# project-codeflare/instaslice

Measured on AMD Instinct MI355X. Metric: pods_scheduled_per_s, higher is better.
Workload: dtype fp32; 1 GPU; model=sleep-pod-partition-allocation, global_batch=698, parallelism=1-controller-shards+1-node-agents, partitioning=static-spx, backend=amdsmi, payload_kernel=False, full=False, cpu_affinity=120-127,248-255, payload_every=0, policy=packed-fit

## Files before the change

__graft_entry__.py:

```python

from __future__ import annotations


def build() -> None:
    import build_native

    build_native.build()

    import instaslice_amd
    import instaslice_amd.agent
    import instaslice_amd.controller
    from instaslice_amd.ops import _payload
    from instaslice_amd.smi import _partitiond

    print("build OK: instaslice_amd + _partitiond + _payload importable")


def smoke() -> None:
    from instaslice_amd.ops import _payload
    from instaslice_amd.runtime.cluster import Cluster
    from instaslice_amd.smi.native import NativeAmdSmi

    ndev = _payload.device_count()
    assert ndev > 0, "smoke() requires a GPU"

    smi = NativeAmdSmi()
    smi.init()
    gpus = smi.list_gpus()
    assert gpus, "no AMD GPUs enumerated via libamd_smi"
    g0 = gpus[0]
    print(
        f"gpu0: {g0.model} uuid={g0.uuid} mem={g0.memory_gb}GB "
        f"mode={g0.compute_mode}/{g0.memory_mode} partitions={len(g0.partitions)}"
    )

    cluster = Cluster(teardown_grace_s=0.0)
    cluster.add_node("smoke-node", smi)
    cluster.start()
    try:
        from instaslice_amd.partition.profiles import ProfileCatalog

        cr = cluster.store.get("Instaslice", "smoke-node", "instaslice-system")
        cat = ProfileCatalog.from_dict(cr["spec"]["placements"])
        profile = next(
            p for p in cat.profiles if p.compute.value == g0.compute_mode
        )
        cluster.submit_pod("smoke-pod", profile.name)
        cluster.wait_pod_scheduled("smoke-pod", timeout=30.0)
        env = cluster.pod_env("smoke-pod")
        device_index = int(env["HIP_VISIBLE_DEVICES"])
        print(f"pod scheduled; partition device_index={device_index} "
              f"uuid={env['ROCR_VISIBLE_DEVICES']}")

        err = _payload.run_vecadd(1 << 22, device=device_index)
        assert err == 0.0, f"vecadd max_err={err}"
        _payload.run_busy(20.0, device=device_index)
        info = _payload.device_info(device_index)
        print(f"payload OK on {info['gcn_arch']}: vecadd exact, "
              f"{info['cu_count']} CUs, {info['xcd_count_visible']} XCD(s) visible")

        cluster.delete_pod("smoke-pod")
        cluster.wait_pod_gone("smoke-pod", timeout=30.0)
        cluster.wait_allocations_empty("smoke-node", timeout=30.0)
    finally:
        cluster.stop()
    print("smoke OK: allocate -> run HIP payload in partition -> teardown")


if __name__ == "__main__":
    import sys

    if len(sys.argv) > 1 and sys.argv[1] == "smoke":
        smoke()
    else:
        build()
```

build_native.py:

```python
#!/usr/bin/env python3

from __future__ import annotations

import os
import subprocess
import sys
import sysconfig
from pathlib import Path

ROOT = Path(__file__).resolve().parent
ROCM = Path(os.environ.get("ROCM_PATH", "/opt/rocm"))
HIPCC = str(ROCM / "bin" / "hipcc")
CLANGXX = str(ROCM / "bin" / "amdclang++")
ARCH = os.environ.get("PYTORCH_ROCM_ARCH", "gfx950")
EXT = sysconfig.get_config_var("EXT_SUFFIX") or ".so"


def pybind_includes() -> list:
    import pybind11

    return [f"-I{pybind11.get_include()}", f"-I{sysconfig.get_paths()['include']}"]


def _srchash(sources: list, cmd_sig: str) -> str:
    import hashlib

    h = hashlib.sha256()
    h.update(cmd_sig.encode())
    for s in sources:
        h.update(Path(s).read_bytes())
    return h.hexdigest()


def newer(target: Path, sources: list, cmd_sig: str = "") -> bool:
    if not target.exists():
        return False
    sidecar = target.with_suffix(target.suffix + ".srchash")
    if not sidecar.exists():
        return False
    return sidecar.read_text().strip() == _srchash(sources, cmd_sig)


def record_hash(target: Path, sources: list, cmd_sig: str = "") -> None:
    sidecar = target.with_suffix(target.suffix + ".srchash")
    sidecar.write_text(_srchash(sources, cmd_sig) + "\n")


def run(cmd: list) -> None:
    print("+", " ".join(str(c) for c in cmd), flush=True)
    subprocess.run([str(c) for c in cmd], check=True, cwd=ROOT)


def build(force: bool = False) -> None:
    smi_dir = ROOT / "instaslice_amd" / "smi"
    ops_dir = ROOT / "instaslice_amd" / "ops"
    bin_dir = ROOT / "instaslice_amd" / "bin"
    bin_dir.mkdir(exist_ok=True)
    (bin_dir / "__init__.py").touch()

    common = ["-O2", "-std=c++17", "-fPIC", f"-I{ROCM}/include",
              f"-L{ROCM}/lib", f"-Wl,-rpath,{ROCM}/lib"]

    src = smi_dir / "csrc" / "partitiond_pybind.cpp"
    hdr = smi_dir / "csrc" / "partitiond_core.hpp"
    out = smi_dir / f"_partitiond{EXT}"
    if force or not newer(out, [src, hdr], "pybind"):
        run([CLANGXX, "-shared", *common, *pybind_includes(), src, "-lamd_smi", "-o", out])
        record_hash(out, [src, hdr], "pybind")

    src = smi_dir / "csrc" / "partitiond_main.cpp"
    out = bin_dir / "partitiond"
    if force or not newer(out, [src, hdr], "daemon"):
        run([CLANGXX, *common, src, "-lamd_smi", "-o", out])
        record_hash(out, [src, hdr], "daemon")

    src = ops_dir / "csrc" / "payload_pybind.hip"
    hdr = ops_dir / "csrc" / "payload_core.hpp"
    hdr_gemm = ops_dir / "csrc" / "payload_gemm.hpp"
    out = ops_dir / f"_payload{EXT}"
    if force or not newer(out, [src, hdr, hdr_gemm], ARCH):
        run([HIPCC, f"--offload-arch={ARCH}", "-shared", *common,
             *pybind_includes(), src, "-o", out])
        record_hash(out, [src, hdr, hdr_gemm], ARCH)

    src = ops_dir / "csrc" / "payload_main.hip"
    out = bin_dir / "instaslice-payload"
    if force or not newer(out, [src, hdr, hdr_gemm], ARCH):
        run([HIPCC, f"--offload-arch={ARCH}", *common, src, "-o", out])
        record_hash(out, [src, hdr, hdr_gemm], ARCH)

    store_dir = ROOT / "instaslice_amd" / "store"
    src = store_dir / "csrc" / "stored_main.cpp"
    hdr2 = store_dir / "csrc" / "msgpack_value.hpp"
    out = bin_dir / "instaslice-stored"
    if force or not newer(out, [src, hdr2], "stored"):
        run(["g++", "-O2", "-std=c++17", "-pthread", src, "-o", out])
        record_hash(out, [src, hdr2], "stored")

    print("native build complete")


if __name__ == "__main__":
    build(force="--force" in sys.argv)
```

instaslice_amd/store/netstore.py:

```python

from __future__ import annotations

import queue
import socket
import socketserver
import struct
import threading
from typing import Callable, List, Optional, Tuple

import msgpack

from instaslice_amd.store.memstore import (
    AlreadyExists,
    Conflict,
    MemStore,
    NotFound,
)
from instaslice_amd.utils import get_logger

_EXC_BY_NAME = {
    "Conflict": Conflict,
    "NotFound": NotFound,
    "AlreadyExists": AlreadyExists,
}

_LEN = struct.Struct(">I")


def _pack(obj: dict) -> bytes:
    payload = msgpack.packb(obj, use_bin_type=True)
    return _LEN.pack(len(payload)) + payload


def _read_msg(rfile) -> Optional[dict]:
    hdr = rfile.read(4)
    if len(hdr) < 4:
        return None
    (n,) = _LEN.unpack(hdr)
    payload = rfile.read(n)
    if len(payload) < n:
        return None
    return msgpack.unpackb(payload, raw=False)


def _execute(store: MemStore, req: dict):
    verb = req.get("verb")
    if verb == "create":
        return store.create(req["obj"])
    if verb == "get":
        return store.get(req["kind"], req["name"], req.get("namespace", ""))
    if verb == "list":
        return store.list(req["kind"], req.get("namespace"))
    if verb == "update":
        return store.update(req["obj"])
    if verb == "delete":
        store.delete(req["kind"], req["name"], req.get("namespace", ""))
        return None
    if verb == "patch":
        return store.patch(req["kind"], req["name"], req.get("namespace", ""),
                           req.get("ops"))
    if verb == "ping":
        return "pong"
    raise ValueError(f"unknown verb {verb!r}")


class _Handler(socketserver.StreamRequestHandler):
    disable_nagle_algorithm = True

    def handle(self) -> None:
        store: MemStore = self.server.store
        log = self.server.log
        wlock = threading.Lock()
        watches = []

        def send(obj: dict) -> None:
            data = _pack(obj)
            with wlock:
                self.wfile.write(data)
                self.wfile.flush()

        def pump_watch(watch_id: int, w) -> None:
            while True:
                ev = w.next(timeout=0.5)
                if ev is None:
                    if w._stopped or self.server.stopping:
                        return
                    continue
                try:
                    send({"watch_id": watch_id, "event": list(ev)})
                except (BrokenPipeError, OSError, ValueError):
                    w.stop()
                    return

        next_watch_id = 0
        try:
            while True:
                req = _read_msg(self.rfile)
                if req is None:
                    break
                rid = req.get("id")
                verb = req.get("verb")
                quiet = req.get("quiet", False)
                try:
                    if verb == "batch":
                        res = store.batch(req["requests"], quiet=quiet)
                    elif verb == "watch":
                        w = store.watch(req.get("kind"), replay=req.get("replay", True),
                                        filters=req.get("filters"),
                                        since=req.get("since"))
                        watches.append(w)
                        next_watch_id += 1
                        wid = next_watch_id
                        send({"id": rid, "ok": True, "result": {
                            "watch_id": wid,
                            "rev": getattr(w, "rev", None),
                            "resumed": getattr(w, "resumed", False)}})
                        threading.Thread(
                            target=pump_watch, args=(wid, w), daemon=True
                        ).start()
                        continue
                    else:
                        res = _execute(store, req)
                        if quiet:
                            res = None
                    send({"id": rid, "ok": True, "result": res})
                except (Conflict, NotFound, AlreadyExists) as e:
                    send({"id": rid, "ok": False,
                          "error": {"type": type(e).__name__, "msg": str(e)}})
                except Exception as e:
                    log.warning("request error: %s", e)
                    send({"id": rid, "ok": False,
                          "error": {"type": "Error", "msg": str(e)}})
        except (ConnectionResetError, BrokenPipeError, OSError):
            pass
        finally:
            for w in watches:
                w.stop()


class StoreServer:

    def __init__(self, store: Optional[MemStore] = None,
                 host: str = "127.0.0.1", port: int = 0) -> None:
        self.store = store or MemStore()
        self.log = get_logger("netstore.server")
        self._srv = socketserver.ThreadingTCPServer((host, port), _Handler,
                                                    bind_and_activate=True)
        self._srv.daemon_threads = True
        self._srv.allow_reuse_address = True
        self._srv.store = self.store
        self._srv.log = self.log
        self._srv.stopping = False
        self.host, self.port = self._srv.server_address
        self._thread = threading.Thread(target=self._srv.serve_forever,
                                        name="netstore-server", daemon=True)

    def start(self) -> "StoreServer":
        self._thread.start()
        return self

    def stop(self) -> None:
        self._srv.stopping = True
        self._srv.shutdown()
        self._srv.server_close()


class _ClientWatch:

    def __init__(self) -> None:
        self._q: "queue.Queue[Optional[Tuple[str, dict]]]" = queue.Queue()
        self._stopped = False
        self.kind: Optional[str] = None
        self._cb = None
        self._cb_lock = threading.Lock()
        self.last_rev: Optional[int] = None

    def set_callback(self, fn) -> None:
        with self._cb_lock:
            while True:
                try:
                    ev = self._q.get_nowait()
                except queue.Empty:
                    break
                if ev is not None:
                    fn(*ev)
            self._cb = fn

    def _deliver(self, event) -> None:
        if self._stopped:
            return
        try:
            rv = int(event[1]["metadata"]["resourceVersion"])
            if self.last_rev is None or rv > self.last_rev:
                self.last_rev = rv
        except (KeyError, TypeError, ValueError, IndexError):
            pass
        with self._cb_lock:
            if self._cb is not None:
                try:
                    self._cb(*event)
                except Exception:
                    import traceback

                    traceback.print_exc()
                return
        self._q.put(event)

    def next(self, timeout: Optional[float] = None) -> Optional[Tuple[str, dict]]:
        try:
            return self._q.get(timeout=timeout)
        except queue.Empty:
            return None

    def stop(self) -> None:
        self._stopped = True
        self._q.put(None)


class NetStoreClient:

    def __init__(self, host: str, port: int, timeout: float = 30.0,
                 reconnect: bool = False,
                 reconnect_backoff_s: float = 0.2) -> None:
        self.host, self.port = host, port
        self._reconnect = reconnect
        self._reconnect_backoff_s = reconnect_backoff_s
        self._sock = socket.create_connection((host, port), timeout=timeout)
        self._sock.settimeout(None)
        self._sock.setsockopt(socket.IPPROTO_TCP, socket.TCP_NODELAY, 1)
        self._rfile = self._sock.makefile("rb")
        self._wlock = threading.Lock()
        self._pending: dict = {}
        self._watches: dict = {}
        self._watch_specs: dict = {}
        self._orphan_events: dict = {}
        self._watch_reg_lock = threading.Lock()
        self._next_id = 0
        self._idlock = threading.Lock()
        self._closed = False
        self.log = get_logger("netstore.client")
        self._reader = threading.Thread(target=self._read_loop,
                                        name="netstore-reader", daemon=True)
        self._reader.start()

    def _dispatch(self, msg: dict) -> None:
        if "watch_id" in msg and "event" in msg:
            wid = msg["watch_id"]
            et, obj = msg["event"]
            with self._watch_reg_lock:
                w = self._watches.get(wid)
                if w is None:
                    self._orphan_events.setdefault(wid, []).append((et, obj))
            if w is not None:
                w._deliver((et, obj))
            return
        ev = self._pending.pop(msg.get("id"), None)
        if ev is not None:
            ev[1] = msg
            ev[0].set()

    def _fail_pending(self, why: str) -> None:
        for rid in list(self._pending):
            ev = self._pending.pop(rid, None)
            if ev is not None:
                ev[1] = {"ok": False, "error": {"type": "Error", "msg": why}}
                ev[0].set()

    def _read_loop(self) -> None:
        while True:
            try:
                while True:
                    msg = _read_msg(self._rfile)
                    if msg is None:
                        break
                    self._dispatch(msg)
            except (OSError, ValueError):
                pass
            self._fail_pending("connection lost")
            if self._closed or not self._reconnect:
                break
            if not self._reconnect_once():
                break
        self._closed = True
        self._fail_pending("connection closed")
        for w in self._watches.values():
            w.stop()

    def _reconnect_once(self) -> bool:
        try:
            self._sock.close()
        except OSError:
            pass
        delay = self._reconnect_backoff_s
        while not self._closed:
            try:
                sock = socket.create_connection((self.host, self.port),
                                                timeout=5.0)
            except OSError:
                import time as _time

                _time.sleep(delay)
                delay = min(delay * 2, 5.0)
                continue
            sock.settimeout(None)
            sock.setsockopt(socket.IPPROTO_TCP, socket.TCP_NODELAY, 1)
            with self._wlock:
                self._sock = sock
                self._rfile = sock.makefile("rb")
            self._fail_pending("connection lost")
            with self._watch_reg_lock:
                live = [(w, spec) for (w, spec) in self._watch_specs.values()
                        if not w._stopped]
                self._watches = {}
            new_specs = {}
            ok = True
            for w, spec in live:
                with self._idlock:
                    self._next_id += 1
                    rid = self._next_id
                resync = dict(spec, replay=True)
                if w.last_rev is not None:
                    resync["since"] = w.last_rev
                try:
                    with self._wlock:
                        self._sock.sendall(_pack({"id": rid, "verb": "watch",
                                                  **resync}))
                    while True:
                        msg = _read_msg(self._rfile)
                        if msg is None:
                            ok = False
                            break
                        if msg.get("id") == rid:
                            new_wid = msg["result"]["watch_id"]
                            with self._watch_reg_lock:
                                self._watches[new_wid] = w
                            new_specs[new_wid] = (w, spec)
                            break
                        self._dispatch(msg)
                except (OSError, ValueError, KeyError):
                    ok = False
                if not ok:
                    break
            if ok:
                with self._watch_reg_lock:
                    self._watch_specs = new_specs
                self.log.warning(
                    "reconnected to store %s:%d (%d watches resynced)",
                    self.host, self.port, len(live))
                return True
            with self._watch_reg_lock:
                self._watches = {}
        return False

    def _call(self, verb: str, **kw):
        if self._closed:
            raise ConnectionError("netstore client closed")
        with self._idlock:
            self._next_id += 1
            rid = self._next_id
        ev = [threading.Event(), None]
        self._pending[rid] = ev
        req = _pack({"id": rid, "verb": verb, **kw})
        try:
            with self._wlock:
                self._sock.sendall(req)
        except OSError as e:
            self._pending.pop(rid, None)
            raise ConnectionError(f"netstore send failed: {e}") from e
        if not ev[0].wait(timeout=60.0):
            self._pending.pop(rid, None)
            raise TimeoutError(f"netstore call {verb} timed out")
        msg = ev[1]
        if msg["ok"]:
            return msg.get("result")
        err = msg["error"]
        if err["type"] == "Error" and "connection" in err["msg"]:
            raise ConnectionError(err["msg"])
        raise _EXC_BY_NAME.get(err["type"], RuntimeError)(err["msg"])


    def create(self, obj: dict) -> dict:
        return self._call("create", obj=obj)

    def get(self, kind: str, name: str, namespace: str = "") -> dict:
        return self._call("get", kind=kind, name=name, namespace=namespace)

    def list(self, kind: str, namespace: Optional[str] = None) -> List[dict]:
        return self._call("list", kind=kind, namespace=namespace)

    def update(self, obj: dict) -> dict:
        return self._call("update", obj=obj)

    def delete(self, kind: str, name: str, namespace: str = "", *, now: float = 0.0) -> None:
        self._call("delete", kind=kind, name=name, namespace=namespace)

    def patch(self, kind: str, name: str, namespace: str = "",
              ops: Optional[List[dict]] = None, *, quiet: bool = False):
        return self._call("patch", kind=kind, name=name, namespace=namespace,
                          ops=ops, quiet=quiet)

    def batch(self, requests: List[dict], *, quiet: bool = False) -> List[dict]:
        return self._call("batch", requests=requests, quiet=quiet)

    def watch(self, kind: Optional[str] = None, *, replay: bool = True,
              filters: Optional[List[dict]] = None):
        w = _ClientWatch()
        w.kind = kind
        spec = {"kind": kind, "replay": replay, "filters": filters}
        res = self._call("watch", kind=kind, replay=replay, filters=filters)
        wid = res["watch_id"]
        if isinstance(res, dict) and res.get("rev") is not None:
            w.last_rev = int(res["rev"])
        with self._watch_reg_lock:
            self._watches[wid] = w
            self._watch_specs[wid] = (w, spec)
            orphans = self._orphan_events.pop(wid, [])
        for ev in orphans:
            w._deliver(ev)
        return w

    def update_with_retry(
        self, kind: str, name: str, namespace: str,
        mutate: Callable[[dict], Optional[dict]], attempts: int = 25,
    ) -> Optional[dict]:
        for attempt in range(attempts):
            try:
                obj = self.get(kind, name, namespace)
            except NotFound:
                return None
            new = mutate(obj)
            if new is None:
                return None
            try:
                return self.update(new)
            except Conflict:
                if attempt >= 2:
                    import random
                    import time as _time

                    _time.sleep(random.random() * 0.002 * attempt)
                continue
        raise Conflict(f"update_with_retry: {attempts} attempts exhausted for {kind}/{name}")

    def close(self) -> None:
        self._closed = True
        try:
            self._sock.close()
        except OSError:
            pass
```

Measured before the change: 1000 pods/s.

## Add native C++ wire client for netstore RPC and event dispatch

Moves the netstore client's socket framing, msgpack encoding, response matching and reader thread into a pybind11 C++ extension. Request/response waits then happen in C++ condition variables instead of Python Events, and events are batched to Python callbacks. It is enabled by default when the extension builds. The aim is to cut Python GIL and per-message overhead on controller/agent store calls. In exchange it adds a new reconnect path and extra concurrency complexity.

New measurement: 1055 pods/s, median of 6. 1.06x the previous value.

```diff
diff --git a/__graft_entry__.py b/__graft_entry__.py
--- a/__graft_entry__.py
+++ b/__graft_entry__.py
@@ -12,8 +12,9 @@
     import instaslice_amd.controller
     from instaslice_amd.ops import _payload
     from instaslice_amd.smi import _partitiond
+    from instaslice_amd.store import _netclient
 
-    print("build OK: instaslice_amd + _partitiond + _payload importable")
+    print("build OK: instaslice_amd + _partitiond + _payload + _netclient importable")
 
 
 def smoke() -> None:
diff --git a/build_native.py b/build_native.py
--- a/build_native.py
+++ b/build_native.py
@@ -97,6 +97,14 @@
         run(["g++", "-O2", "-std=c++17", "-pthread", src, "-o", out])
         record_hash(out, [src, hdr2], "stored")
 
+    src = store_dir / "csrc" / "netclient_pybind.cpp"
+    hdr3 = store_dir / "csrc" / "netclient_core.hpp"
+    out = store_dir / f"_netclient{EXT}"
+    if force or not newer(out, [src, hdr3], "netclient"):
+        run(["g++", "-O2", "-std=c++17", "-fPIC", "-shared", "-pthread",
+             "-fvisibility=hidden", *pybind_includes(), src, "-o", out])
+        record_hash(out, [src, hdr3], "netclient")
+
     print("native build complete")
 
 
diff --git a/instaslice_amd/store/csrc/netclient_core.hpp b/instaslice_amd/store/csrc/netclient_core.hpp
--- /dev/null
+++ b/instaslice_amd/store/csrc/netclient_core.hpp
@@ -0,0 +1,489 @@
+
+#pragma once
+
+#include <sys/socket.h>
+#include <sys/types.h>
+
+#include <atomic>
+#include <cerrno>
+#include <chrono>
+#include <condition_variable>
+#include <cstdint>
+#include <cstring>
+#include <memory>
+#include <mutex>
+#include <string>
+#include <thread>
+#include <unordered_map>
+#include <utility>
+#include <vector>
+
+namespace netclient {
+
+constexpr uint32_t kMaxFrame = 64u << 20;
+
+
+struct Peek {
+  enum Kind { Response, Event, Other, Bad };
+  Kind kind = Bad;
+  uint64_t id = 0;
+};
+
+class Scanner {
+ public:
+  Scanner(const uint8_t* p, size_t n) : p_(p), end_(p + n) {}
+
+  bool at_end() const { return p_ == end_; }
+
+  bool skip() {
+    uint64_t todo = 1;
+    while (todo > 0) {
+      --todo;
+      if (p_ >= end_) return false;
+      uint8_t c = *p_++;
+      uint64_t n = 0;
+      if (c < 0x80 || c >= 0xe0) continue;
+      if ((c & 0xf0) == 0x80) { n = 2ull * (c & 0x0f); goto container; }
+      if ((c & 0xf0) == 0x90) { n = c & 0x0f; goto container; }
+      if ((c & 0xe0) == 0xa0) { if (!advance(c & 0x1f)) return false; continue; }
+      switch (c) {
+        case 0xc0: case 0xc2: case 0xc3: continue;
+        case 0xc4: case 0xd9: if (!take_be(1, n) || !advance(n)) return false; continue;
+        case 0xc5: case 0xda: if (!take_be(2, n) || !advance(n)) return false; continue;
+        case 0xc6: case 0xdb: if (!take_be(4, n) || !advance(n)) return false; continue;
+        case 0xca: case 0xce: case 0xd2: if (!advance(4)) return false; continue;
+        case 0xcb: case 0xcf: case 0xd3: if (!advance(8)) return false; continue;
+        case 0xcc: case 0xd0: if (!advance(1)) return false; continue;
+        case 0xcd: case 0xd1: if (!advance(2)) return false; continue;
+        case 0xdc: if (!take_be(2, n)) return false; goto container;
+        case 0xdd: if (!take_be(4, n)) return false; goto container;
+        case 0xde: if (!take_be(2, n)) return false; n *= 2; goto container;
+        case 0xdf: if (!take_be(4, n)) return false; n *= 2; goto container;
+        default: return false;
+      }
+    container:
+      todo += n;
+      if (todo > static_cast<uint64_t>(end_ - p_)) return false;
+    }
+    return true;
+  }
+
+  bool take_map(uint64_t& n) {
+    if (p_ >= end_) return false;
+    uint8_t c = *p_;
+    if ((c & 0xf0) == 0x80) { ++p_; n = c & 0x0f; return true; }
+    if (c == 0xde) { ++p_; return take_be(2, n); }
+    if (c == 0xdf) { ++p_; return take_be(4, n); }
+    return false;
+  }
+
+  bool take_str(const uint8_t*& s, size_t& len) {
+    if (p_ >= end_) return false;
+    uint8_t c = *p_;
+    uint64_t n = 0;
+    const uint8_t* save = p_;
+    if ((c & 0xe0) == 0xa0) { ++p_; n = c & 0x1f; }
+    else if (c == 0xd9) { ++p_; if (!take_be(1, n)) { p_ = save; return false; } }
+    else if (c == 0xda) { ++p_; if (!take_be(2, n)) { p_ = save; return false; } }
+    else if (c == 0xdb) { ++p_; if (!take_be(4, n)) { p_ = save; return false; } }
+    else return false;
+    if (static_cast<uint64_t>(end_ - p_) < n) { p_ = save; return false; }
+    s = p_;
+    len = static_cast<size_t>(n);
+    p_ += n;
+    return true;
+  }
+
+  bool take_uint(uint64_t& v) {
+    if (p_ >= end_) return false;
+    uint8_t c = *p_;
+    const uint8_t* save = p_;
+    if (c < 0x80) { ++p_; v = c; return true; }
+    int w = c == 0xcc ? 1 : c == 0xcd ? 2 : c == 0xce ? 4 : c == 0xcf ? 8 : 0;
+    int sw = c == 0xd0 ? 1 : c == 0xd1 ? 2 : c == 0xd2 ? 4 : c == 0xd3 ? 8 : 0;
+    if (w) {
+      ++p_;
+      if (!take_be(w, v)) { p_ = save; return false; }
+      return true;
+    }
+    if (sw) {
+      ++p_;
+      uint64_t raw;
+      if (!take_be(sw, raw)) { p_ = save; return false; }
+      if ((raw >> (8 * sw - 1)) & 1) { p_ = save; return false; }
+      v = raw;
+      return true;
+    }
+    return false;
+  }
+
+ private:
+  bool advance(uint64_t n) {
+    if (static_cast<uint64_t>(end_ - p_) < n) return false;
+    p_ += n;
+    return true;
+  }
+  bool take_be(int n, uint64_t& v) {
+    if (end_ - p_ < n) return false;
+    v = 0;
+    for (int k = 0; k < n; ++k) v = (v << 8) | *p_++;
+    return true;
+  }
+
+  const uint8_t* p_;
+  const uint8_t* end_;
+};
+
+inline Peek peek_frame(const uint8_t* p, size_t n) {
+  Peek out;
+  Scanner sc(p, n);
+  uint64_t pairs = 0;
+  if (!sc.take_map(pairs)) {
+    out.kind = (sc.skip() && sc.at_end()) ? Peek::Other : Peek::Bad;
+    return out;
+  }
+  bool has_id = false, has_wid = false, has_event = false;
+  uint64_t id = 0, wid = 0;
+  for (uint64_t k = 0; k < pairs; ++k) {
+    const uint8_t* s = nullptr;
+    size_t len = 0;
+    if (sc.take_str(s, len)) {
+      if (len == 2 && std::memcmp(s, "id", 2) == 0) {
+        uint64_t v;
+        if (sc.take_uint(v)) { has_id = true; id = v; continue; }
+        has_id = false;
+      } else if (len == 8 && std::memcmp(s, "watch_id", 8) == 0) {
+        uint64_t v;
+        if (sc.take_uint(v)) { has_wid = true; wid = v; continue; }
+        has_wid = false;
+      } else if (len == 5 && std::memcmp(s, "event", 5) == 0) {
+        has_event = true;
+      }
+    } else if (!sc.skip()) {
+      return out;
+    }
+    if (!sc.skip()) return out;
+  }
+  if (!sc.at_end()) return out;
+  if (has_wid && has_event) { out.kind = Peek::Event; out.id = wid; }
+  else if (has_id) { out.kind = Peek::Response; out.id = id; }
+  else out.kind = Peek::Other;
+  return out;
+}
+
+
+struct EventSink {
+  virtual ~EventSink() = default;
+  virtual bool on_events(std::vector<std::string>& frames) = 0;
+  virtual void on_lost(const char* why) = 0;
+};
+
+enum class Status { Ok, Pending, Timeout, Lost, Closed, SendFailed };
+
+inline const char* status_message(Status s) {
+  switch (s) {
+    case Status::Lost: return "connection lost";
+    case Status::Closed: return "connection closed";
+    case Status::Timeout: return "timed out";
+    case Status::SendFailed: return "send failed";
+    default: return "";
+  }
+}
+
+class Wire : public std::enable_shared_from_this<Wire> {
+  struct Waiter {
+    std::condition_variable cv;
+    bool done = false;
+    Status st = Status::Pending;
+    std::string frame;
+  };
+
+ public:
+  struct Stats {
+    uint64_t responses = 0;
+    uint64_t events = 0;
+    uint64_t dropped = 0;
+    uint64_t batches = 0;
+  };
+
+  static std::shared_ptr<Wire> create(int fd, std::shared_ptr<EventSink> sink) {
+    return std::shared_ptr<Wire>(new Wire(fd, std::move(sink)));
+  }
+
+  Wire(const Wire&) = delete;
+  Wire& operator=(const Wire&) = delete;
+
+  ~Wire() {
+    if (reader_.joinable()) {
+      if (reader_.get_id() == std::this_thread::get_id()) reader_.detach();
+      else reader_.join();
+    }
+  }
+
+  void start() {
+    std::lock_guard<std::mutex> g(join_mu_);
+    if (started_) return;
+    started_ = true;
+    auto self = shared_from_this();
+    reader_ = std::thread([self] { self->run(); });
+  }
+
+  class Call {
+   public:
+    Call(Wire& w, uint64_t id) : w_(w), id_(id) {
+      std::lock_guard<std::mutex> g(w_.mu_);
+      if (w_.lost_) {
+        wt_.done = true;
+        wt_.st = w_.lost_status_;
+      } else {
+        registered_ = w_.pending_.emplace(id_, &wt_).second;
+        if (!registered_) {
+          wt_.done = true;
+          wt_.st = Status::SendFailed;
+          err_ = EINVAL;
+        }
+      }
+    }
+    ~Call() {
+      if (!registered_) return;
+      std::lock_guard<std::mutex> g(w_.mu_);
+      auto it = w_.pending_.find(id_);
+      if (it != w_.pending_.end() && it->second == &wt_) w_.pending_.erase(it);
+    }
+    Call(const Call&) = delete;
+    Call& operator=(const Call&) = delete;
+
+    Status send(const char* data, size_t n) {
+      {
+        std::lock_guard<std::mutex> g(w_.mu_);
+        if (wt_.done) return wt_.st;
+      }
+      int e = w_.send_all(data, n);
+      if (e == 0) return Status::Ok;
+      std::lock_guard<std::mutex> g(w_.mu_);
+      if (wt_.done && wt_.st != Status::Ok) return wt_.st;
+      if (e < 0) return w_.stopping_.load() ? Status::Closed : Status::Lost;
+      err_ = e;
+      return Status::SendFailed;
+    }
+
+    Status wait_for(std::chrono::nanoseconds slice) {
+      std::unique_lock<std::mutex> g(w_.mu_);
+      if (!wt_.done) {
+#if defined(__SANITIZE_THREAD__)
+        wt_.cv.wait_until(g, std::chrono::system_clock::now() + slice,
+                          [&] { return wt_.done; });
+#else
+        wt_.cv.wait_for(g, slice, [&] { return wt_.done; });
+#endif
+      }
+      return wt_.done ? wt_.st : Status::Pending;
+    }
+
+    std::string& frame() { return wt_.frame; }
+    int send_errno() const { return err_; }
+
+   private:
+    Wire& w_;
+    uint64_t id_;
+    Waiter wt_;
+    bool registered_ = false;
+    int err_ = 0;
+  };
+
+  Status call(const std::string& framed_request, uint64_t id, double timeout_s,
+              std::string* response) {
+    Call c(*this, id);
+    Status st = c.send(framed_request.data(), framed_request.size());
+    if (st != Status::Ok) return st;
+    auto deadline = std::chrono::steady_clock::now() +
+                    std::chrono::duration_cast<std::chrono::nanoseconds>(
+                        std::chrono::duration<double>(timeout_s));
+    for (;;) {
+      auto now = std::chrono::steady_clock::now();
+      if (now >= deadline) return Status::Timeout;
+      st = c.wait_for(deadline - now);
+      if (st == Status::Pending) continue;
+      if (st == Status::Ok && response) *response = std::move(c.frame());
+      return st;
+    }
+  }
+
+  void stop() {
+    if (!stopping_.exchange(true))
+      ::shutdown(fd_, SHUT_RDWR);
+    {
+      std::lock_guard<std::mutex> g(write_mu_);
+      fd_dead_ = true;
+    }
+    bool joined = false;
+    {
+      std::lock_guard<std::mutex> g(join_mu_);
+      if (!started_) {
+        started_ = true;
+        joined = true;
+      } else if (reader_.joinable() &&
+                 reader_.get_id() != std::this_thread::get_id()) {
+        reader_.join();
+        joined = true;
+      }
+    }
+    if (joined) fail_all(Status::Closed);
+  }
+
+  void abort_connection() {
+    std::lock_guard<std::mutex> g(write_mu_);
+    if (!fd_dead_) ::shutdown(fd_, SHUT_RDWR);
+  }
+
+  bool alive() const {
+    std::lock_guard<std::mutex> g(mu_);
+    return !lost_;
+  }
+
+  Stats stats() const {
+    Stats s;
+    s.responses = responses_.load(std::memory_order_relaxed);
+    s.events = events_.load(std::memory_order_relaxed);
+    s.dropped = dropped_.load(std::memory_order_relaxed);
+    s.batches = batches_.load(std::memory_order_relaxed);
+    return s;
+  }
+
+  size_t pending() const {
+    std::lock_guard<std::mutex> g(mu_);
+    return pending_.size();
+  }
+
+ private:
+  Wire(int fd, std::shared_ptr<EventSink> sink) : fd_(fd), sink_(std::move(sink)) {}
+
+  int send_all(const char* p, size_t left) {
+    std::lock_guard<std::mutex> g(write_mu_);
+    if (fd_dead_) return -1;
+    while (left > 0) {
+      ssize_t n = ::send(fd_, p, left, MSG_NOSIGNAL);
+      if (n < 0) {
+        if (errno == EINTR) continue;
+        return errno ? errno : EIO;
+      }
+      p += n;
+      left -= static_cast<size_t>(n);
+    }
+    return 0;
+  }
+
+  void complete(uint64_t id, const uint8_t* p, size_t n) {
+    std::lock_guard<std::mutex> g(mu_);
+    auto it = pending_.find(id);
+    if (it == pending_.end()) {
+      dropped_.fetch_add(1, std::memory_order_relaxed);
+      return;
+    }
+    Waiter* w = it->second;
+    pending_.erase(it);
+    w->frame.assign(reinterpret_cast<const char*>(p), n);
+    w->st = Status::Ok;
+    w->done = true;
+    w->cv.notify_one();
+    responses_.fetch_add(1, std::memory_order_relaxed);
+  }
+
+  void fail_all(Status st) {
+    std::lock_guard<std::mutex> g(mu_);
+    if (!lost_) {
+      lost_ = true;
+      lost_status_ = st;
+    }
+    for (auto& kv : pending_) {
+      kv.second->st = st;
+      kv.second->done = true;
+      kv.second->cv.notify_one();
+    }
+    pending_.clear();
+  }
+
+  void run() {
+    std::vector<char> buf(64 * 1024);
+    size_t rd = 0, wr = 0;
+    std::vector<std::string> events;
+    while (!stopping_.load()) {
+      if (wr == buf.size()) {
+        if (rd > 0) {
+          std::memmove(buf.data(), buf.data() + rd, wr - rd);
+          wr -= rd;
+          rd = 0;
+        } else {
+          buf.resize(buf.size() * 2);
+        }
+      }
+      ssize_t n = ::recv(fd_, buf.data() + wr, buf.size() - wr, 0);
+      if (n < 0 && errno == EINTR) continue;
+      if (n <= 0) break;
+      wr += static_cast<size_t>(n);
+
+      bool bad = false;
+      while (wr - rd >= 4) {
+        const uint8_t* h = reinterpret_cast<const uint8_t*>(buf.data() + rd);
+        uint32_t len = (static_cast<uint32_t>(h[0]) << 24) | (static_cast<uint32_t>(h[1]) << 16) |
+                       (static_cast<uint32_t>(h[2]) << 8) | static_cast<uint32_t>(h[3]);
+        if (len > kMaxFrame) { bad = true; break; }
+        size_t need = 4 + static_cast<size_t>(len);
+        if (wr - rd < need) {
+          if (buf.size() - rd < need) {
+            std::memmove(buf.data(), buf.data() + rd, wr - rd);
+            wr -= rd;
+            rd = 0;
+            if (buf.size() < need) buf.resize(need);
+          }
+          break;
+        }
+        const uint8_t* f = h + 4;
+        Peek pk = peek_frame(f, len);
+        if (pk.kind == Peek::Response) complete(pk.id, f, len);
+        else if (pk.kind == Peek::Event) events.emplace_back(reinterpret_cast<const char*>(f), len);
+        else if (pk.kind == Peek::Other) dropped_.fetch_add(1, std::memory_order_relaxed);
+        else { bad = true; break; }
+        rd += need;
+      }
+      if (!events.empty()) {
+        events_.fetch_add(events.size(), std::memory_order_relaxed);
+        batches_.fetch_add(1, std::memory_order_relaxed);
+        bool ok = sink_ ? sink_->on_events(events) : true;
+        events.clear();
+        if (!ok) bad = true;
+      }
+      if (bad) break;
+      if (rd == wr) {
+        rd = wr = 0;
+        if (buf.size() > (1u << 20)) {
+          buf.resize(64 * 1024);
+          buf.shrink_to_fit();
+        }
+      }
+    }
+    bool closed = stopping_.load();
+    fail_all(closed ? Status::Closed : Status::Lost);
+    if (sink_) sink_->on_lost(status_message(closed ? Status::Closed : Status::Lost));
+  }
+
+  const int fd_;
+  std::shared_ptr<EventSink> sink_;
+
+  mutable std::mutex mu_;
+  std::unordered_map<uint64_t, Waiter*> pending_;
+  bool lost_ = false;
+  Status lost_status_ = Status::Lost;
+
+  std::mutex write_mu_;
+  bool fd_dead_ = false;
+
+  std::mutex join_mu_;
+  bool started_ = false;
+  std::thread reader_;
+  std::atomic<bool> stopping_{false};
+
+  std::atomic<uint64_t> responses_{0}, events_{0}, dropped_{0}, batches_{0};
+};
+
+}
diff --git a/instaslice_amd/store/csrc/netclient_pybind.cpp b/instaslice_amd/store/csrc/netclient_pybind.cpp
--- /dev/null
+++ b/instaslice_amd/store/csrc/netclient_pybind.cpp
@@ -0,0 +1,475 @@
+
+#include <pybind11/pybind11.h>
+
+#include <string>
+#include <vector>
+
+#include "netclient_core.hpp"
+
+namespace py = pybind11;
+using netclient::Status;
+using netclient::Wire;
+
+namespace {
+
+
+constexpr int kMaxDepth = 511;
+
+inline void put_be(std::string& out, uint64_t v, int n) {
+  for (int s = 8 * (n - 1); s >= 0; s -= 8) out.push_back(static_cast<char>(v >> s));
+}
+
+inline void put_uint(std::string& out, uint64_t n) {
+  if (n < 0x80) out.push_back(static_cast<char>(n));
+  else if (n <= 0xff) { out.push_back(static_cast<char>(0xcc)); put_be(out, n, 1); }
+  else if (n <= 0xffff) { out.push_back(static_cast<char>(0xcd)); put_be(out, n, 2); }
+  else if (n <= 0xffffffffULL) { out.push_back(static_cast<char>(0xce)); put_be(out, n, 4); }
+  else { out.push_back(static_cast<char>(0xcf)); put_be(out, n, 8); }
+}
+
+inline void put_int(std::string& out, int64_t v) {
+  if (v >= 0) { put_uint(out, static_cast<uint64_t>(v)); return; }
+  uint64_t u = static_cast<uint64_t>(v);
+  if (v >= -32) out.push_back(static_cast<char>(v));
+  else if (v >= INT8_MIN) { out.push_back(static_cast<char>(0xd0)); put_be(out, u, 1); }
+  else if (v >= INT16_MIN) { out.push_back(static_cast<char>(0xd1)); put_be(out, u, 2); }
+  else if (v >= INT32_MIN) { out.push_back(static_cast<char>(0xd2)); put_be(out, u, 4); }
+  else { out.push_back(static_cast<char>(0xd3)); put_be(out, u, 8); }
+}
+
+bool encode_obj(PyObject* o, std::string& out, int depth) {
+  if (o == Py_None) { out.push_back(static_cast<char>(0xc0)); return true; }
+  if (o == Py_True) { out.push_back(static_cast<char>(0xc3)); return true; }
+  if (o == Py_False) { out.push_back(static_cast<char>(0xc2)); return true; }
+  if (PyUnicode_CheckExact(o)) {
+    Py_ssize_t n = 0;
+    const char* s = PyUnicode_AsUTF8AndSize(o, &n);
+    if (!s) { PyErr_Clear(); return false; }
+    if (n < 32) out.push_back(static_cast<char>(0xa0 | n));
+    else if (n <= 0xff) { out.push_back(static_cast<char>(0xd9)); put_be(out, n, 1); }
+    else if (n <= 0xffff) { out.push_back(static_cast<char>(0xda)); put_be(out, n, 2); }
+    else if (static_cast<uint64_t>(n) <= 0xffffffffULL) { out.push_back(static_cast<char>(0xdb)); put_be(out, n, 4); }
+    else return false;
+    out.append(s, static_cast<size_t>(n));
+    return true;
+  }
+  if (PyLong_CheckExact(o)) {
+    int overflow = 0;
+    long long v = PyLong_AsLongLongAndOverflow(o, &overflow);
+    if (overflow == 0) {
+      if (v == -1 && PyErr_Occurred()) { PyErr_Clear(); return false; }
+      put_int(out, v);
+      return true;
+    }
+    if (overflow < 0) return false;
+    unsigned long long u = PyLong_AsUnsignedLongLong(o);
+    if (u == static_cast<unsigned long long>(-1) && PyErr_Occurred()) { PyErr_Clear(); return false; }
+    put_uint(out, u);
+    return true;
+  }
+  if (PyDict_CheckExact(o)) {
+    if (depth >= kMaxDepth) return false;
+    Py_ssize_t n = PyDict_Size(o);
+    if (n < 16) out.push_back(static_cast<char>(0x80 | n));
+    else if (n <= 0xffff) { out.push_back(static_cast<char>(0xde)); put_be(out, n, 2); }
+    else if (static_cast<uint64_t>(n) <= 0xffffffffULL) { out.push_back(static_cast<char>(0xdf)); put_be(out, n, 4); }
+    else return false;
+    Py_ssize_t pos = 0;
+    PyObject *k, *v;
+    while (PyDict_Next(o, &pos, &k, &v)) {
+      if (!encode_obj(k, out, depth + 1)) return false;
+      if (!encode_obj(v, out, depth + 1)) return false;
+    }
+    return true;
+  }
+  if (PyList_CheckExact(o) || PyTuple_CheckExact(o)) {
+    if (depth >= kMaxDepth) return false;
+    bool is_list = PyList_CheckExact(o);
+    Py_ssize_t n = is_list ? PyList_GET_SIZE(o) : PyTuple_GET_SIZE(o);
+    if (n < 16) out.push_back(static_cast<char>(0x90 | n));
+    else if (n <= 0xffff) { out.push_back(static_cast<char>(0xdc)); put_be(out, n, 2); }
+    else if (static_cast<uint64_t>(n) <= 0xffffffffULL) { out.push_back(static_cast<char>(0xdd)); put_be(out, n, 4); }
+    else return false;
+    for (Py_ssize_t i = 0; i < n; ++i) {
+      PyObject* e = is_list ? PyList_GET_ITEM(o, i) : PyTuple_GET_ITEM(o, i);
+      if (!encode_obj(e, out, depth + 1)) return false;
+    }
+    return true;
+  }
+  if (PyFloat_CheckExact(o)) {
+    double d = PyFloat_AS_DOUBLE(o);
+    uint64_t bits;
+    static_assert(sizeof(bits) == sizeof(d), "double size");
+    std::memcpy(&bits, &d, sizeof(bits));
+    out.push_back(static_cast<char>(0xcb));
+    put_be(out, bits, 8);
+    return true;
+  }
+  if (PyBytes_CheckExact(o)) {
+    Py_ssize_t n = PyBytes_GET_SIZE(o);
+    if (n <= 0xff) { out.push_back(static_cast<char>(0xc4)); put_be(out, n, 1); }
+    else if (n <= 0xffff) { out.push_back(static_cast<char>(0xc5)); put_be(out, n, 2); }
+    else if (static_cast<uint64_t>(n) <= 0xffffffffULL) { out.push_back(static_cast<char>(0xc6)); put_be(out, n, 4); }
+    else return false;
+    out.append(PyBytes_AS_STRING(o), static_cast<size_t>(n));
+    return true;
+  }
+  return false;
+}
+
+void encode_into(py::handle o, std::string& out) {
+  size_t mark = out.size();
+  if (encode_obj(o.ptr(), out, 0)) return;
+  out.resize(mark);
+  static py::object* packb = nullptr;
+  if (!packb) packb = new py::object(py::module_::import("msgpack").attr("packb"));
+  py::object b = (*packb)(o, py::arg("use_bin_type") = true);
+  char* p = nullptr;
+  Py_ssize_t n = 0;
+  if (PyBytes_AsStringAndSize(b.ptr(), &p, &n) != 0) throw py::error_already_set();
+  out.append(p, static_cast<size_t>(n));
+}
+
+
+struct Decoder {
+  const uint8_t* p;
+  const uint8_t* end;
+
+  PyObject* fail(const char* what) {
+    PyErr_SetString(PyExc_ValueError, what);
+    return nullptr;
+  }
+
+  bool take_be(int n, uint64_t& v) {
+    if (end - p < n) { fail("msgpack: incomplete input"); return false; }
+    v = 0;
+    for (int k = 0; k < n; ++k) v = (v << 8) | *p++;
+    return true;
+  }
+
+  PyObject* take_str(uint64_t n) {
+    if (static_cast<uint64_t>(end - p) < n) return fail("msgpack: incomplete input");
+    PyObject* s = PyUnicode_DecodeUTF8(reinterpret_cast<const char*>(p),
+                                       static_cast<Py_ssize_t>(n), nullptr);
+    p += n;
+    return s;
+  }
+
+  PyObject* take_bin(uint64_t n) {
+    if (static_cast<uint64_t>(end - p) < n) return fail("msgpack: incomplete input");
+    PyObject* b = PyBytes_FromStringAndSize(reinterpret_cast<const char*>(p),
+                                            static_cast<Py_ssize_t>(n));
+    p += n;
+    return b;
+  }
+
+  PyObject* take_arr(uint64_t n, int depth) {
+    if (static_cast<uint64_t>(end - p) < n) return fail("msgpack: incomplete input");
+    PyObject* l = PyList_New(static_cast<Py_ssize_t>(n));
+    if (!l) return nullptr;
+    for (uint64_t k = 0; k < n; ++k) {
+      PyObject* e = next(depth + 1);
+      if (!e) { Py_DECREF(l); return nullptr; }
+      PyList_SET_ITEM(l, static_cast<Py_ssize_t>(k), e);
+    }
+    return l;
+  }
+
+  PyObject* take_map(uint64_t n, int depth) {
+    if (static_cast<uint64_t>(end - p) / 2 < n) return fail("msgpack: incomplete input");
+    PyObject* d = PyDict_New();
+    if (!d) return nullptr;
+    for (uint64_t k = 0; k < n; ++k) {
+      PyObject* key = next(depth + 1);
+      if (!key) { Py_DECREF(d); return nullptr; }
+      if (!PyUnicode_CheckExact(key) && !PyBytes_CheckExact(key)) {
+        PyErr_Format(PyExc_ValueError, "%.100s is not allowed for map key",
+                     Py_TYPE(key)->tp_name);
+        Py_DECREF(key);
+        Py_DECREF(d);
+        return nullptr;
+      }
+      PyObject* val = next(depth + 1);
+      if (!val) { Py_DECREF(key); Py_DECREF(d); return nullptr; }
+      int rc = PyDict_SetItem(d, key, val);
+      Py_DECREF(key);
+      Py_DECREF(val);
+      if (rc != 0) { Py_DECREF(d); return nullptr; }
+    }
+    return d;
+  }
+
+  PyObject* next(int depth) {
+    if (depth > kMaxDepth) return fail("msgpack: nesting too deep");
+    if (p >= end) return fail("msgpack: incomplete input");
+    uint8_t c = *p++;
+    uint64_t n = 0;
+    if (c < 0x80) return PyLong_FromLong(c);
+    if (c >= 0xe0) return PyLong_FromLong(static_cast<int8_t>(c));
+    if ((c & 0xf0) == 0x80) return take_map(c & 0x0f, depth);
+    if ((c & 0xf0) == 0x90) return take_arr(c & 0x0f, depth);
+    if ((c & 0xe0) == 0xa0) return take_str(c & 0x1f);
+    switch (c) {
+      case 0xc0: Py_RETURN_NONE;
+      case 0xc2: Py_RETURN_FALSE;
+      case 0xc3: Py_RETURN_TRUE;
+      case 0xc4: return take_be(1, n) ? take_bin(n) : nullptr;
+      case 0xc5: return take_be(2, n) ? take_bin(n) : nullptr;
+      case 0xc6: return take_be(4, n) ? take_bin(n) : nullptr;
+      case 0xca: {
+        if (!take_be(4, n)) return nullptr;
+        uint32_t bits = static_cast<uint32_t>(n);
+        float f;
+        std::memcpy(&f, &bits, sizeof(f));
+        return PyFloat_FromDouble(f);
+      }
+      case 0xcb: {
+        if (!take_be(8, n)) return nullptr;
+        double d;
+        std::memcpy(&d, &n, sizeof(d));
+        return PyFloat_FromDouble(d);
+      }
+      case 0xcc: return take_be(1, n) ? PyLong_FromUnsignedLongLong(n) : nullptr;
+      case 0xcd: return take_be(2, n) ? PyLong_FromUnsignedLongLong(n) : nullptr;
+      case 0xce: return take_be(4, n) ? PyLong_FromUnsignedLongLong(n) : nullptr;
+      case 0xcf: return take_be(8, n) ? PyLong_FromUnsignedLongLong(n) : nullptr;
+      case 0xd0: return take_be(1, n) ? PyLong_FromLong(static_cast<int8_t>(n)) : nullptr;
+      case 0xd1: return take_be(2, n) ? PyLong_FromLong(static_cast<int16_t>(n)) : nullptr;
+      case 0xd2: return take_be(4, n) ? PyLong_FromLong(static_cast<int32_t>(n)) : nullptr;
+      case 0xd3: return take_be(8, n) ? PyLong_FromLongLong(static_cast<int64_t>(n)) : nullptr;
+      case 0xd9: return take_be(1, n) ? take_str(n) : nullptr;
+      case 0xda: return take_be(2, n) ? take_str(n) : nullptr;
+      case 0xdb: return take_be(4, n) ? take_str(n) : nullptr;
+      case 0xdc: return take_be(2, n) ? take_arr(n, depth) : nullptr;
+      case 0xdd: return take_be(4, n) ? take_arr(n, depth) : nullptr;
+      case 0xde: return take_be(2, n) ? take_map(n, depth) : nullptr;
+      case 0xdf: return take_be(4, n) ? take_map(n, depth) : nullptr;
+      default: return fail("msgpack: ext types are not supported");
+    }
+  }
+};
+
+PyObject* decode_raw(const char* data, size_t n) {
+  Decoder d{reinterpret_cast<const uint8_t*>(data), reinterpret_cast<const uint8_t*>(data) + n};
+  PyObject* o = d.next(0);
+  if (o && d.p != d.end) {
+    Py_DECREF(o);
+    return d.fail("msgpack: extra data after the message");
+  }
+  return o;
+}
+
+
+inline bool interpreter_usable() {
+#if PY_VERSION_HEX >= 0x030D0000
+  return Py_IsInitialized() && !Py_IsFinalizing();
+#else
+  return Py_IsInitialized() && !_Py_IsFinalizing();
+#endif
+}
+
+class PySink : public netclient::EventSink {
+ public:
+  PySink(py::object on_events, py::object on_lost)
+      : on_events_(on_events.release().ptr()), on_lost_(on_lost.release().ptr()) {}
+
+  ~PySink() override {
+    if (!on_events_ && !on_lost_) return;
+    if (!interpreter_usable()) return;
+    PyGILState_STATE st = PyGILState_Ensure();
+    Py_CLEAR(on_events_);
+    Py_CLEAR(on_lost_);
+    PyGILState_Release(st);
+  }
+
+  void release() {
+    Py_CLEAR(on_events_);
+    Py_CLEAR(on_lost_);
+  }
+
+  bool on_events(std::vector<std::string>& frames) override {
+    if (!interpreter_usable()) return false;
+    PyGILState_STATE st = PyGILState_Ensure();
+    gil_.fetch_add(1, std::memory_order_relaxed);
+    bool ok = true;
+    PyObject* cb = on_events_;
+    if (cb) {
+      Py_INCREF(cb);
+      PyObject* list = PyList_New(0);
+      for (auto& f : frames) {
+        PyObject* msg = list ? decode_raw(f.data(), f.size()) : nullptr;
+        if (!msg) { ok = false; break; }
+        int rc = PyList_Append(list, msg);
+        Py_DECREF(msg);
+        if (rc != 0) { ok = false; break; }
+      }
+      if (!ok) PyErr_Clear();
+      if (list && PyList_GET_SIZE(list) > 0) {
+        PyObject* r = PyObject_CallFunctionObjArgs(cb, list, nullptr);
+        if (!r) PyErr_WriteUnraisable(cb);
+        Py_XDECREF(r);
+      }
+      Py_XDECREF(list);
+      Py_DECREF(cb);
+    }
+    PyGILState_Release(st);
+    return ok;
+  }
+
+  void on_lost(const char* why) override {
+    if (!interpreter_usable()) return;
+    PyGILState_STATE st = PyGILState_Ensure();
+    gil_.fetch_add(1, std::memory_order_relaxed);
+    PyObject* cb = on_lost_;
+    if (cb) {
+      Py_INCREF(cb);
+      PyObject* r = PyObject_CallFunction(cb, "s", why);
+      if (!r) PyErr_WriteUnraisable(cb);
+      Py_XDECREF(r);
+      Py_DECREF(cb);
+    }
+    PyGILState_Release(st);
+  }
+
+  uint64_t gil_acquisitions() const { return gil_.load(std::memory_order_relaxed); }
+
+ private:
+  PyObject* on_events_;
+  PyObject* on_lost_;
+  std::atomic<uint64_t> gil_{0};
+};
+
+
+class PyWire {
+ public:
+  PyWire(int fd, py::object on_events, py::object on_lost)
+      : sink_(std::make_shared<PySink>(std::move(on_events), std::move(on_lost))),
+        wire_(Wire::create(fd, sink_)) {
+    wire_->start();
+  }
+
+  ~PyWire() {
+    py::gil_scoped_release nogil;
+    wire_->stop();
+  }
+
+  py::object call(py::handle request, uint64_t id, double timeout_s) {
+    std::string req(4, '\0');
+    encode_into(request, req);
+    size_t n = req.size() - 4;
+    if (n > netclient::kMaxFrame) throw py::value_error("netstore request over the 64 MiB frame limit");
+    req[0] = static_cast<char>(n >> 24);
+    req[1] = static_cast<char>(n >> 16);
+    req[2] = static_cast<char>(n >> 8);
+    req[3] = static_cast<char>(n);
+
+    Wire::Call c(*wire_, id);
+    Status st;
+    bool interrupted = false;
+    {
+      py::gil_scoped_release nogil;
+      st = c.send(req.data(), req.size());
+      if (st == Status::Ok) {
+        auto deadline = std::chrono::steady_clock::now() +
+                        std::chrono::duration_cast<std::chrono::nanoseconds>(
+                            std::chrono::duration<double>(timeout_s));
+        const auto slice = std::chrono::milliseconds(100);
+        for (;;) {
+          auto now = std::chrono::steady_clock::now();
+          if (now >= deadline) { st = Status::Timeout; break; }
+          auto left = deadline - now;
+          st = c.wait_for(left < slice ? left : std::chrono::nanoseconds(slice));
+          if (st != Status::Pending) break;
+          py::gil_scoped_acquire gil;
+          if (PyErr_CheckSignals() != 0) { interrupted = true; break; }
+        }
+      }
+    }
+    if (interrupted) throw py::error_already_set();
+    switch (st) {
+      case Status::Ok: {
+        PyObject* msg = decode_raw(c.frame().data(), c.frame().size());
+        if (!msg) {
+          PyErr_Clear();
+          wire_->abort_connection();
+          PyErr_SetString(PyExc_ConnectionError, "connection lost");
+          throw py::error_already_set();
+        }
+        return py::reinterpret_steal<py::object>(msg);
+      }
+      case Status::Timeout:
+        PyErr_SetString(PyExc_TimeoutError, "timed out");
+        throw py::error_already_set();
+      case Status::SendFailed: {
+        std::string m = std::string("netstore send failed: ") + std::strerror(c.send_errno());
+        PyErr_SetString(PyExc_ConnectionError, m.c_str());
+        throw py::error_already_set();
+      }
+      default:
+        PyErr_SetString(PyExc_ConnectionError, netclient::status_message(st));
+        throw py::error_already_set();
+    }
+  }
+
+  void stop() {
+    {
+      py::gil_scoped_release nogil;
+      wire_->stop();
+    }
+    sink_->release();
+  }
+
+  bool alive() const { return wire_->alive(); }
+
+  py::dict stats() const {
+    Wire::Stats s = wire_->stats();
+    py::dict d;
+    d["responses"] = s.responses;
+    d["events"] = s.events;
+    d["event_batches"] = s.batches;
+    d["dropped"] = s.dropped;
+    d["reader_gil_acquisitions"] = sink_->gil_acquisitions();
+    d["pending"] = wire_->pending();
+    return d;
+  }
+
+ private:
+  std::shared_ptr<PySink> sink_;
+  std::shared_ptr<Wire> wire_;
+};
+
+}
+
+PYBIND11_MODULE(_netclient, m) {
+  m.doc() = "Native wire for NetStoreClient: reader thread, call/wait, msgpack codec";
+
+  m.def("encode", [](py::handle obj) {
+    std::string out;
+    encode_into(obj, out);
+    return py::bytes(out);
+  }, py::arg("obj"), "msgpack.packb(obj, use_bin_type=True), byte for byte");
+
+  m.def("decode", [](py::bytes data) {
+    char* p = nullptr;
+    Py_ssize_t n = 0;
+    if (PyBytes_AsStringAndSize(data.ptr(), &p, &n) != 0) throw py::error_already_set();
+    PyObject* o = decode_raw(p, static_cast<size_t>(n));
+    if (!o) throw py::error_already_set();
+    return py::reinterpret_steal<py::object>(o);
+  }, py::arg("data"), "msgpack.unpackb(data, raw=False)");
+
+  m.attr("MAX_FRAME") = py::int_(netclient::kMaxFrame);
+
+  py::class_<PyWire>(m, "Wire")
+      .def(py::init<int, py::object, py::object>(), py::arg("fd"),
+           py::arg("on_events"), py::arg("on_lost"),
+           "Start a reader on a connected blocking socket fd (borrowed).\n"
+           "on_events(list_of_message_dicts) and on_lost(why) run on the reader thread.")
+      .def("call", &PyWire::call, py::arg("request"), py::arg("id"), py::arg("timeout"),
+           "Send one request dict and return the response dict.\n"
+           "Raises TimeoutError, or ConnectionError when the connection is lost or closed.")
+      .def("stop", &PyWire::stop,
+           "Stop and join the reader; pending calls fail with ConnectionError.")
+      .def("alive", &PyWire::alive)
+      .def("stats", &PyWire::stats);
+}
diff --git a/instaslice_amd/store/netstore.py b/instaslice_amd/store/netstore.py
--- a/instaslice_amd/store/netstore.py
+++ b/instaslice_amd/store/netstore.py
@@ -1,6 +1,7 @@
 
 from __future__ import annotations
 
+import os
 import queue
 import socket
 import socketserver
@@ -17,6 +18,17 @@
     NotFound,
 )
 from instaslice_amd.utils import get_logger
+
+try:
+    from instaslice_amd.store import _netclient
+except ImportError:
+    _netclient = None
+
+
+def _native_wire_wanted() -> bool:
+    return (_netclient is not None
+            and os.environ.get("INSTASLICE_NATIVE_CLIENT", "1") != "0")
+
 
 _EXC_BY_NAME = {
     "Conflict": Conflict,
@@ -228,20 +240,151 @@
         self._sock = socket.create_connection((host, port), timeout=timeout)
         self._sock.settimeout(None)
         self._sock.setsockopt(socket.IPPROTO_TCP, socket.TCP_NODELAY, 1)
-        self._rfile = self._sock.makefile("rb")
         self._wlock = threading.Lock()
         self._pending: dict = {}
         self._watches: dict = {}
         self._watch_specs: dict = {}
         self._orphan_events: dict = {}
-        self._watch_reg_lock = threading.Lock()
+        self._watch_reg_lock = threading.RLock()
         self._next_id = 0
         self._idlock = threading.Lock()
         self._closed = False
         self.log = get_logger("netstore.client")
-        self._reader = threading.Thread(target=self._read_loop,
-                                        name="netstore-reader", daemon=True)
-        self._reader.start()
+        self._wire = None
+        self._wire_gen = 0
+        self._rc_lock = threading.Lock()
+        self._reconnecting = False
+        if _native_wire_wanted():
+            self._rfile = None
+            self._reader = None
+            with self._rc_lock:
+                self._wire = self._new_wire(self._sock)
+        else:
+            self._rfile = self._sock.makefile("rb")
+            self._reader = threading.Thread(target=self._read_loop,
+                                            name="netstore-reader", daemon=True)
+            self._reader.start()
+
+    @property
+    def wire(self) -> str:
+        return "native" if self._wire is not None else "python"
+
+    def stats(self) -> dict:
+        wire = self._wire
+        return dict(wire.stats()) if wire is not None else {}
+
+
+    def _new_wire(self, sock):
+        self._wire_gen += 1
+        gen = self._wire_gen
+        return _netclient.Wire(
+            sock.fileno(), self._on_wire_events,
+            lambda why, g=gen: self._on_wire_lost(g, why))
+
+    def _on_wire_events(self, msgs: list) -> None:
+        for msg in msgs:
+            self._dispatch(msg)
+
+    def _on_wire_lost(self, gen: int, why: str) -> None:
+        with self._rc_lock:
+            if gen != self._wire_gen or self._reconnecting:
+                return
+            final = self._closed or not self._reconnect
+            if not final:
+                self._reconnecting = True
+        if final:
+            self._finish_native()
+            return
+        threading.Thread(target=self._reconnect_native,
+                         name="netstore-reconnect", daemon=True).start()
+
+    def _finish_native(self) -> None:
+        self._closed = True
+        with self._watch_reg_lock:
+            watches = list(self._watches.values())
+            watches += [w for (w, _spec) in self._watch_specs.values()
+                        if w not in watches]
+        for w in watches:
+            if not w._stopped:
+                w.stop()
+
+    def _reconnect_native(self) -> None:
+        import time as _time
+
+        delay = self._reconnect_backoff_s
+        while True:
+            with self._rc_lock:
+                if self._closed:
+                    self._reconnecting = False
+                    break
+                old_wire, old_sock = self._wire, self._sock
+            old_wire.stop()
+            try:
+                old_sock.close()
+            except OSError:
+                pass
+            try:
+                sock = socket.create_connection((self.host, self.port),
+                                                timeout=5.0)
+            except OSError:
+                _time.sleep(delay)
+                delay = min(delay * 2, 5.0)
+                continue
+            sock.settimeout(None)
+            sock.setsockopt(socket.IPPROTO_TCP, socket.TCP_NODELAY, 1)
+            with self._watch_reg_lock:
+                live = [(w, spec) for (w, spec) in self._watch_specs.values()
+                        if not w._stopped]
+                self._watches = {}
+                self._orphan_events = {}
+            with self._rc_lock:
+                if self._closed:
+                    self._reconnecting = False
+                    sock.close()
+                    break
+                self._sock = sock
+                self._wire = wire = self._new_wire(sock)
+            new_specs = {}
+            ok = True
+            for w, spec in live:
+                with self._idlock:
+                    self._next_id += 1
+                    rid = self._next_id
+                resync = dict(spec, replay=True)
+                if w.last_rev is not None:
+                    resync["since"] = w.last_rev
+                try:
+                    msg = wire.call({"id": rid, "verb": "watch", **resync},
+                                    rid, 60.0)
+                    new_wid = msg["result"]["watch_id"]
+                except (OSError, ValueError, KeyError, TypeError):
+                    ok = False
+                    break
+                with self._watch_reg_lock:
+                    self._watches[new_wid] = w
+                    for ev in self._orphan_events.pop(new_wid, []):
+                        w._deliver(ev)
+                new_specs[new_wid] = (w, spec)
+            if ok:
+                with self._watch_reg_lock:
+                    self._watch_specs = new_specs
+                with self._rc_lock:
+                    done = wire.alive() or self._closed
+                    if done:
+                        self._reconnecting = False
+                if done:
+                    self.log.warning(
+                        "reconnected to store %s:%d (%d watches resynced)",
+                        self.host, self.port, len(live))
+                    if not self._closed:
+                        return
+                    break
+            else:
+                with self._watch_reg_lock:
+                    self._watches = {}
+                _time.sleep(self._reconnect_backoff_s)
+        self._finish_native()
+
 
     def _dispatch(self, msg: dict) -> None:
         if "watch_id" in msg and "event" in msg:
@@ -358,6 +501,18 @@
         with self._idlock:
             self._next_id += 1
             rid = self._next_id
+        wire = self._wire
+        if wire is not None:
+            try:
+                msg = wire.call({"id": rid, "verb": verb, **kw}, rid, 60.0)
+            except TimeoutError:
+                raise TimeoutError(f"netstore call {verb} timed out") from None
+            if msg["ok"]:
+                return msg.get("result")
+            err = msg["error"]
+            if err["type"] == "Error" and "connection" in err["msg"]:
+                raise ConnectionError(err["msg"])
+            raise _EXC_BY_NAME.get(err["type"], RuntimeError)(err["msg"])
         ev = [threading.Event(), None]
         self._pending[rid] = ev
         req = _pack({"id": rid, "verb": verb, **kw})
@@ -414,9 +569,8 @@
         with self._watch_reg_lock:
             self._watches[wid] = w
             self._watch_specs[wid] = (w, spec)
-            orphans = self._orphan_events.pop(wid, [])
-        for ev in orphans:
-            w._deliver(ev)
+            for ev in self._orphan_events.pop(wid, []):
+                w._deliver(ev)
         return w
 
     def update_with_retry(
@@ -444,6 +598,16 @@
 
     def close(self) -> None:
         self._closed = True
+        if self._wire is not None:
+            with self._rc_lock:
+                wire, sock = self._wire, self._sock
+            wire.stop()
+            try:
+                sock.close()
+            except OSError:
+                pass
+            self._finish_native()
+            return
         try:
             self._sock.close()
         except OSError:
```
